# a-r-r-o-w/finetrainers

Measured on NVIDIA H100. Metric: latent_tokens_per_sec, higher is better.
Workload: dtype bf16

## Files before the change

finetrainers_b200/csrc/b2d_attn.cu:

```cuda
#include <stdlib.h>
#include <type_traits>
#include "b2d_internal.h"
#include "b2d_ptx.cuh"

namespace b2d {

constexpr int ATT_THREADS = 384;
constexpr int TILE = 128;
constexpr int PANEL = 64;
constexpr int TILE_PANEL_BYTES = TILE * PANEL * 2;
constexpr int HALF_PANEL_BYTES = 64 * PANEL * 2;
constexpr int ATT_SMEM_LIMIT = 227 * 1024;
constexpr float LOG2E = 1.4426950408889634f;
constexpr float LN2 = 0.6931471805599453f;

template <int HD>
struct AttnShape {
    static_assert(HD == 64 || HD == 128, "attention is built for head_dim 64 and 128");
    static constexpr int PANELS = HD / PANEL;
    static constexpr int TILE_BYTES = PANELS * TILE_PANEL_BYTES;
    static constexpr int HALF_BYTES = PANELS * HALF_PANEL_BYTES;
};

__device__ __forceinline__ float fast_exp2(float x) {
// ... 271 lines not shown
    const long long t = (long long)blockIdx.x * blockDim.x + threadIdx.x;
    const long long total = (long long)B * Sq * H * LANES;
    const bool ok = t < total;
    const long long e0 = (ok ? t : 0) * 8;
    uint4 a = *reinterpret_cast<const uint4*>(out + e0);
    uint4 d = *reinterpret_cast<const uint4*>(dout + e0);
    float acc = bf16_lo(a.x) * bf16_lo(d.x) + bf16_hi(a.x) * bf16_hi(d.x) + bf16_lo(a.y) * bf16_lo(d.y) +
                bf16_hi(a.y) * bf16_hi(d.y) + bf16_lo(a.z) * bf16_lo(d.z) + bf16_hi(a.z) * bf16_hi(d.z) +
                bf16_lo(a.w) * bf16_lo(d.w) + bf16_hi(a.w) * bf16_hi(d.w);
#pragma unroll
    for (int o = 1; o < LANES; o <<= 1) acc += __shfl_xor_sync(0xffffffffu, acc, o);
    if (ok && (t & (LANES - 1)) == 0) {
        const long long hr = t >> LOG2_LANES;
        const int h = (int)(hr % H);
        const long long bq = hr / H;
        const int q = (int)(bq % Sq);
        const int b = (int)(bq / Sq);
        const long long o = ((long long)b * H + h) * Sq + q;
        delta[o] = acc;
        nlse2[o] = -lse[o] * LOG2E;
    }
}

struct AttnBwdParams {
    CUtensorMap tmX1, tmX2, tmY1, tmY2;
    const float* key_bias;
    const float* delta;
    const float* nlse2;
    __nv_bfloat16* out1;
    __nv_bfloat16* out2;
    float* acc1;
    float* acc2;
    long long part_stride;
    int y_per_split;
    int B, H, Sq, Sk;
    float scale, scale_log2;
};

constexpr int BWD_STAGES = 4;
constexpr int ATT_MAX_SPLITS = 8;
template <int HD>
constexpr int BWD_SMEM = 2 * AttnShape<HD>::TILE_BYTES + BWD_STAGES * 2 * AttnShape<HD>::HALF_BYTES + 1024 + 256;
static_assert(BWD_SMEM<64> <= ATT_SMEM_LIMIT && BWD_SMEM<128> <= ATT_SMEM_LIMIT, "attn_bwd shared memory");
template <int HD>
constexpr int BWD_REGS_PRODUCER = HD == 64 ? 40 : 24;
template <int HD>
constexpr int BWD_REGS_MATH = HD == 64 ? 232 : 240;
static_assert(BWD_REGS_PRODUCER<64> * 128 + BWD_REGS_MATH<64> * 256 == 168 * ATT_THREADS &&
                  BWD_REGS_PRODUCER<128> * 128 + BWD_REGS_MATH<128> * 256 == 168 * ATT_THREADS,
              "setmaxnreg split");

template <bool DKV, int HD>
__global__ void __launch_bounds__(ATT_THREADS, 1) attn_bwd_kernel(const __grid_constant__ AttnBwdParams p) {
    constexpr int TILE_BYTES = AttnShape<HD>::TILE_BYTES, HALF_BYTES = AttnShape<HD>::HALF_BYTES;
    griddep_launch_dependents();
    extern __shared__ uint8_t smem_raw[];
    uint8_t* smem = reinterpret_cast<uint8_t*>((reinterpret_cast<uintptr_t>(smem_raw) + 1023) & ~uintptr_t(1023));
    uint8_t* sX = smem;
    uint8_t* sY = smem + 2 * TILE_BYTES;
    uint64_t* x_bar = reinterpret_cast<uint64_t*>(sY + BWD_STAGES * 2 * HALF_BYTES);
    uint64_t* full_bar = x_bar + 1;
    uint64_t* empty_bar = full_bar + BWD_STAGES;

    const int warp = threadIdx.x >> 5, lane = threadIdx.x & 31;
    const int xt = blockIdx.x, bh = blockIdx.y;
    const int b = bh / p.H, h = bh % p.H;
    const int S_x = DKV ? p.Sk : p.Sq, S_y = DKV ? p.Sq : p.Sk;
    const int n_y = (S_y + 63) / 64;
    const int y_begin = blockIdx.z * p.y_per_split;
    const int y_end = min(n_y, y_begin + p.y_per_split);

    if (threadIdx.x == 0) {
        tma_prefetch_desc(&p.tmX1);
        tma_prefetch_desc(&p.tmX2);
        tma_prefetch_desc(&p.tmY1);
        tma_prefetch_desc(&p.tmY2);
        mbar_init(x_bar, 1);
        for (int i = 0; i < BWD_STAGES; ++i) {
            mbar_init(&full_bar[i], 1);
            mbar_init(&empty_bar[i], 256);
        }
        fence_mbar_init();
    }
    __syncthreads();
    griddep_wait();

    if (warp < 4) {
        setmaxnreg_dec<BWD_REGS_PRODUCER<HD>>();
        if (warp == 0 && elect_one()) {
            mbar_expect_tx(x_bar, 2 * TILE_BYTES);
            tma_load_tile<HD, TILE_PANEL_BYTES>(sX, &p.tmX1, x_bar, h, xt * TILE, b);
            tma_load_tile<HD, TILE_PANEL_BYTES>(sX + TILE_BYTES, &p.tmX2, x_bar, h, xt * TILE, b);
            int stage = 0;
            uint32_t phase = 0;
            for (int y = y_begin; y < y_end; ++y) {
                mbar_wait(&empty_bar[stage], phase ^ 1);
                uint8_t* s1 = sY + stage * 2 * HALF_BYTES;
                mbar_expect_tx(&full_bar[stage], 2 * HALF_BYTES);
                tma_load_tile<HD, HALF_PANEL_BYTES>(s1, &p.tmY1, &full_bar[stage], h, y * 64, b);
                tma_load_tile<HD, HALF_PANEL_BYTES>(s1 + HALF_BYTES, &p.tmY2, &full_bar[stage], h, y * 64, b);
                if (++stage == BWD_STAGES) {
                    stage = 0;
                    phase ^= 1;
                }
            }
        }
        return;
    }
    setmaxnreg_inc<BWD_REGS_MATH<HD>>();
    const int cw = (warp >> 2) - 1, wq = warp & 3;
    const int qd = lane & 3;
    const uint32_t x1 = smem_u32(sX) + cw * HALF_PANEL_BYTES, x2 = x1 + TILE_BYTES;
    const float* kb = p.key_bias ? p.key_bias + (long long)b * p.Sk : nullptr;
    const float* nlse2 = p.nlse2 + (long long)bh * p.Sq;
    const float* delta = p.delta + (long long)bh * p.Sq;
    const int nq = p.B * p.H * p.Sq;
    auto neg_lse2 = [&](int q) { return HD == 64 ? nlse2[q] : delta[q + nq]; };
    const float sl2 = p.scale_log2;
    const int r0 = xt * TILE + cw * 64 + wq * 16 + (lane >> 2);

    float row_off[2], row_delta[2];
#pragma unroll
    for (int hh = 0; hh < 2; ++hh) {
        const int r = r0 + 8 * hh;
        if (DKV) {
            row_off[hh] = (kb != nullptr && r < p.Sk) ? kb[r] * LOG2E : 0.f;
            row_delta[hh] = 0.f;
        } else {
            row_off[hh] = r < p.Sq ? neg_lse2(r) : 0.f;
            row_delta[hh] = r < p.Sq ? delta[r] : 0.f;
        }
    }
    float acc1[HD / 2], acc2[HD / 2];
#pragma unroll
    for (int i = 0; i < HD / 2; ++i) acc1[i] = acc2[i] = 0.f;
    float c_off[16], c_delta[16];
    auto load_cols = [&](int y) {
#pragma unroll
        for (int k = 0; k < 16; ++k) {
            const int c = y * 64 + 8 * (k >> 1) + 2 * qd + (k & 1);
            const bool ok = c < S_y;
            if (DKV) {
                c_off[k] = ok ? neg_lse2(c) : 0.f;
                c_delta[k] = ok ? delta[c] : 0.f;
            } else {
                c_off[k] = (ok && kb != nullptr) ? kb[c] * LOG2E : 0.f;
            }
        }
    };
    float s[32], dp[32];
    auto elementwise = [&](int y, auto ragged) {
#pragma unroll
        for (int k = 0; k < 16; ++k) {
            const int jj = k >> 1, e = k & 1;
            const bool ok = !decltype(ragged)::value || y * 64 + 8 * jj + 2 * qd + e < S_y;
#pragma unroll
            for (int hh = 0; hh < 2; ++hh) {
                const int i = 4 * jj + 2 * hh + e;
                const float pr = ok ? fast_exp2(fmaf(s[i], sl2, row_off[hh] + c_off[k])) : 0.f;
                const float dl = DKV ? c_delta[k] : row_delta[hh];
                s[i] = pr;
                dp[i] = pr * (dp[i] - dl);
            }
        }
    };
    auto turn_begin = [&] { named_bar_sync(1 + cw, 256); };
    auto turn_end = [&](bool last) {
        if (cw == 0 || !last) named_bar_arrive(2 - cw, 256);
    };
    mbar_wait(x_bar, 0);
    if (cw == 1) named_bar_arrive(1, 256);
    int stage = 0;
    uint32_t phase = 0;
    for (int y = y_begin; y < y_end; ++y) {
        mbar_wait(&full_bar[stage], phase);
        const uint32_t y1 = smem_u32(sY + stage * 2 * HALF_BYTES), y2 = y1 + HALF_BYTES;
        turn_begin();
        wgmma_fence();
        mma_xyt<64, HD, TILE_PANEL_BYTES, HALF_PANEL_BYTES>(s, x1, y1);
        mma_xyt<64, HD, TILE_PANEL_BYTES, HALF_PANEL_BYTES>(dp, x2, y2);
        wgmma_commit();
        turn_end(false);
        if (HD == 64) load_cols(y);
        wgmma_wait<0>();
        wgmma_fence_regs(s);
        wgmma_fence_regs(dp);
        if (HD != 64) load_cols(y);
        if ((y + 1) * 64 > S_y)
            elementwise(y, std::true_type{});
        else
            elementwise(y, std::false_type{});
        uint32_t pa[4][4], da[4][4];
        acc_to_a<4>(dp, da);
        turn_begin();
        wgmma_fence();
        if (DKV) {
            acc_to_a<4>(s, pa);
            mma_az<4, HD, HALF_PANEL_BYTES>(acc1, pa, y2);
            mma_az<4, HD, HALF_PANEL_BYTES>(acc2, da, y1);
        } else {
            mma_az<4, HD, HALF_PANEL_BYTES>(acc2, da, y1);
        }
        wgmma_commit();
        turn_end(y + 1 == y_end);
        wgmma_wait<0>();
        wgmma_fence_regs(acc1);
        wgmma_fence_regs(acc2);
        mbar_arrive(&empty_bar[stage]);
        if (++stage == BWD_STAGES) {
            stage = 0;
            phase ^= 1;
        }
    }
#pragma unroll
    for (int hh = 0; hh < 2; ++hh) {
        const int r = r0 + 8 * hh;
        if (r >= S_x) continue;
        const long long base = ((long long)bh * S_x + r) * HD;
#pragma unroll
        for (int jj = 0; jj < HD / 8; ++jj) {
            const int c = 8 * jj + 2 * qd, i = 4 * jj + 2 * hh;
            const float g0 = acc2[i] * p.scale, g1 = acc2[i + 1] * p.scale;
            if (p.acc2 != nullptr) {
                const long long zoff = (long long)blockIdx.z * p.part_stride;
                *reinterpret_cast<float2*>(p.acc2 + zoff + base + c) = make_float2(g0, g1);
                if (DKV) *reinterpret_cast<float2*>(p.acc1 + zoff + base + c) = make_float2(acc1[i], acc1[i + 1]);
            } else {
                *reinterpret_cast<uint32_t*>(p.out2 + base + c) = pack_bf16x2(g0, g1);
                if (DKV) *reinterpret_cast<uint32_t*>(p.out1 + base + c) = pack_bf16x2(acc1[i], acc1[i + 1]);
            }
        }
    }
}

__global__ void attn_dkv_reduce_kernel(const float* __restrict__ part, int splits, long long stride, long long n,
                                       __nv_bfloat16* __restrict__ dv, __nv_bfloat16* __restrict__ dk) {
    griddep_launch_dependents();
    griddep_wait();
    const long long i = ((long long)blockIdx.x * blockDim.x + threadIdx.x) * 4;
    if (i + 3 >= 2 * n) return;
    float4 a = *reinterpret_cast<const float4*>(part + i);
    for (int z = 1; z < splits; ++z) {
        const float4 v = *reinterpret_cast<const float4*>(part + z * stride + i);
        a.x += v.x;
        a.y += v.y;
        a.z += v.z;
        a.w += v.w;
    }
    __nv_bfloat16* dst = i < n ? dv + i : dk + (i - n);
    *reinterpret_cast<uint2*>(dst) = make_uint2(pack_bf16x2(a.x, a.y), pack_bf16x2(a.z, a.w));
}

static int make_head_map(CUtensorMap* m, const void* base, int hd, int B, int H, int S, long long stride_h,
                         long long stride_s, long long stride_b, int box_rows = 128) {
// ... 21 lines not shown
    return 0;
}

template <int HD>
static int attn_fwd(const void* q, const void* k, const void* v, const float* key_bias, void* out, float* lse, int B,
                    int H, int Sq, int Sk, float scale, cudaStream_t st) {
    AttnFwdParams p;
    memset(&p, 0, sizeof(p));
    int rc;
    if ((rc = make_head_map(&p.tmQ, q, HD, B, H, Sq, (long long)Sq * HD, HD, (long long)H * Sq * HD))) return rc;
    if ((rc = make_head_map(&p.tmK, k, HD, B, H, Sk, (long long)Sk * HD, HD, (long long)H * Sk * HD))) return rc;
    if ((rc = make_head_map(&p.tmV, v, HD, B, H, Sk, (long long)Sk * HD, HD, (long long)H * Sk * HD))) return rc;
    p.key_bias = key_bias;
    p.out = (__nv_bfloat16*)out;
    p.lse = lse;
    p.B = B; p.H = H; p.Sq = Sq; p.Sk = Sk;
    p.scale_log2 = scale * LOG2E;
    if ((rc = set_smem((const void*)attn_fwd_kernel<HD>, FWD_SMEM<HD>, "attn_fwd"))) return rc;
    launch_k(attn_fwd_kernel<HD>, dim3((Sq + TILE - 1) / TILE, B * H), dim3(ATT_THREADS), FWD_SMEM<HD>, st, p);
    B2D_CHECK_LAUNCH("attn_fwd");
    return 0;
}

template <int HD>
static int attn_bwd(const void* q, const void* k, const void* v, const float* key_bias, const void* out,
                    const void* dout, const float* lse, float* delta_ws, void* dq, void* dk, void* dv, int B, int H,
                    int Sq, int Sk, float scale, cudaStream_t st) {
    {
        long long total = (long long)B * Sq * H * (HD / 8);
        launch_k(attn_delta_kernel<HD>, dim3((unsigned)((total + 255) / 256)), dim3(256), 0, st,
                 (const __nv_bfloat16*)out, (const __nv_bfloat16*)dout, lse, delta_ws, delta_ws + (long long)B * H * Sq,
                 B, H, Sq);
        B2D_CHECK_LAUNCH("attn_delta");
    }
    CUtensorMap mQ, mK, mV, mdO, mQy, mKy, mVy, mdOy;
    int rc;
    const long long hs_q = (long long)Sq * HD, hs_k = (long long)Sk * HD, tok = (long long)H * HD;
    if ((rc = make_head_map(&mQ, q, HD, B, H, Sq, hs_q, HD, H * hs_q))) return rc;
    if ((rc = make_head_map(&mK, k, HD, B, H, Sk, hs_k, HD, H * hs_k))) return rc;
    if ((rc = make_head_map(&mV, v, HD, B, H, Sk, hs_k, HD, H * hs_k))) return rc;
    if ((rc = make_head_map(&mdO, dout, HD, B, H, Sq, HD, tok, Sq * tok))) return rc;
    if ((rc = make_head_map(&mQy, q, HD, B, H, Sq, hs_q, HD, H * hs_q, 64))) return rc;
    if ((rc = make_head_map(&mKy, k, HD, B, H, Sk, hs_k, HD, H * hs_k, 64))) return rc;
    if ((rc = make_head_map(&mVy, v, HD, B, H, Sk, hs_k, HD, H * hs_k, 64))) return rc;
    if ((rc = make_head_map(&mdOy, dout, HD, B, H, Sq, HD, tok, Sq * tok, 64))) return rc;
    if ((rc = set_smem((const void*)attn_bwd_kernel<true, HD>, BWD_SMEM<HD>, "attn_bwd_dkv"))) return rc;
    if ((rc = set_smem((const void*)attn_bwd_kernel<false, HD>, BWD_SMEM<HD>, "attn_bwd_dq"))) return rc;
    AttnBwdParams p;
    memset(&p, 0, sizeof(p));
    p.key_bias = key_bias; p.delta = delta_ws; p.nlse2 = delta_ws + (long long)B * H * Sq;
    p.B = B; p.H = H; p.Sq = Sq; p.Sk = Sk;
    p.scale = scale; p.scale_log2 = scale * LOG2E;
    p.tmX1 = mK; p.tmX2 = mV; p.tmY1 = mQy; p.tmY2 = mdOy;
    p.out1 = (__nv_bfloat16*)dv; p.out2 = (__nv_bfloat16*)dk;
    const int n_yq = (Sq + 63) / 64;
    const int kv_ctas = ((Sk + TILE - 1) / TILE) * B * H;
    const int nsm = device_sm_count();
    if (nsm <= 0) return B2D_ERR_CUDA;
    int splits = 1;
    if (Sk <= 512 && kv_ctas < nsm && n_yq >= 8) splits = min(ATT_MAX_SPLITS, min(n_yq / 4, (nsm + kv_ctas - 1) / kv_ctas));
    p.y_per_split = (n_yq + splits - 1) / splits;
    splits = (n_yq + p.y_per_split - 1) / p.y_per_split;
    if (splits > 1) {
        const long long n_kv = (long long)B * H * Sk * HD;
        p.acc1 = delta_ws + 2LL * B * H * Sq;
        p.acc2 = p.acc1 + n_kv;
        p.part_stride = 2 * n_kv;
        launch_k(attn_bwd_kernel<true, HD>, dim3((Sk + TILE - 1) / TILE, B * H, splits), dim3(ATT_THREADS), BWD_SMEM<HD>,
                 st, p);
        B2D_CHECK_LAUNCH("attn_bwd_dkv(split)");
        launch_k(attn_dkv_reduce_kernel, dim3((unsigned)((2 * n_kv / 4 + 255) / 256)), dim3(256), 0, st, (const float*)p.acc1,
                 splits, 2 * n_kv, n_kv, (__nv_bfloat16*)dv, (__nv_bfloat16*)dk);
        B2D_CHECK_LAUNCH("attn_bwd_dkv(reduce)");
    } else {
        launch_k(attn_bwd_kernel<true, HD>, dim3((Sk + TILE - 1) / TILE, B * H), dim3(ATT_THREADS), BWD_SMEM<HD>, st, p);
        B2D_CHECK_LAUNCH("attn_bwd_dkv");
    }
    p.acc1 = p.acc2 = nullptr;
    p.tmX1 = mQ; p.tmX2 = mdO; p.tmY1 = mKy; p.tmY2 = mVy;
    p.out1 = nullptr; p.out2 = (__nv_bfloat16*)dq;
    p.y_per_split = (Sk + 63) / 64;
    launch_k(attn_bwd_kernel<false, HD>, dim3((Sq + TILE - 1) / TILE, B * H), dim3(ATT_THREADS), BWD_SMEM<HD>, st, p);
    B2D_CHECK_LAUNCH("attn_bwd_dq");
    return 0;
}

}

using namespace b2d;

extern "C" int b2d_attn_fwd_hd(const void* q, const void* k, const void* v, const float* key_bias, void* out, float* lse,
                               int32_t B, int32_t H, int32_t Sq, int32_t Sk, int32_t head_dim, float scale,
                               void* stream) {
    B2D_BIND(q);
    if (B <= 0 || H <= 0 || Sq <= 0 || Sk <= 0) return set_error(B2D_ERR_SHAPE, "attn_fwd: bad dims");
    if (head_dim != 64 && head_dim != 128)
        return set_error(B2D_ERR_SHAPE, "attn_fwd: head_dim %d is not supported (64 or 128)", (int)head_dim);
    if (reinterpret_cast<uintptr_t>(out) & 31) return set_error(B2D_ERR_ALIGN, "attn_fwd: out must be 32-byte aligned");
    cudaStream_t st = reinterpret_cast<cudaStream_t>(stream);
    return head_dim == 64 ? b2d::attn_fwd<64>(q, k, v, key_bias, out, lse, B, H, Sq, Sk, scale, st)
                          : b2d::attn_fwd<128>(q, k, v, key_bias, out, lse, B, H, Sq, Sk, scale, st);
}

extern "C" int b2d_attn_bwd_hd(const void* q, const void* k, const void* v, const float* key_bias, const void* out,
                               const void* dout, const float* lse, float* delta_ws, void* dq, void* dk, void* dv,
                               int32_t B, int32_t H, int32_t Sq, int32_t Sk, int32_t head_dim, float scale,
                               void* stream) {
    B2D_BIND(q);
    if (B <= 0 || H <= 0 || Sq <= 0 || Sk <= 0) return set_error(B2D_ERR_SHAPE, "attn_bwd: bad dims");
    if (head_dim != 64 && head_dim != 128)
        return set_error(B2D_ERR_SHAPE, "attn_bwd: head_dim %d is not supported (64 or 128)", (int)head_dim);
    cudaStream_t st = reinterpret_cast<cudaStream_t>(stream);
    return head_dim == 64
               ? b2d::attn_bwd<64>(q, k, v, key_bias, out, dout, lse, delta_ws, dq, dk, dv, B, H, Sq, Sk, scale, st)
               : b2d::attn_bwd<128>(q, k, v, key_bias, out, dout, lse, delta_ws, dq, dk, dv, B, H, Sq, Sk, scale, st);
}

extern "C" int b2d_attn_fwd(const void* q, const void* k, const void* v, const float* key_bias, void* out, float* lse,
                            int32_t B, int32_t H, int32_t Sq, int32_t Sk, float scale, void* stream) {
    return b2d_attn_fwd_hd(q, k, v, key_bias, out, lse, B, H, Sq, Sk, 64, scale, stream);
}

extern "C" int b2d_attn_bwd(const void* q, const void* k, const void* v, const float* key_bias, const void* out,
                            const void* dout, const float* lse, float* delta_ws, void* dq, void* dk, void* dv,
                            int32_t B, int32_t H, int32_t Sq, int32_t Sk, float scale, void* stream) {
    return b2d_attn_bwd_hd(q, k, v, key_bias, out, dout, lse, delta_ws, dq, dk, dv, B, H, Sq, Sk, 64, scale, stream);
}
```

finetrainers_b200/lib.py:

```python
from __future__ import annotations

import ctypes as C
import os
import subprocess
import threading

_HERE = os.path.dirname(os.path.abspath(__file__))
LIB_PATH = os.path.join(_HERE, "libb2d.so")
_lib = None
_lock = threading.Lock()


class B2DError(RuntimeError):
    pass


class GemmDesc(C.Structure):
    _fields_ = [
        ("A", C.c_void_p), ("lda", C.c_int64),
        ("B", C.c_void_p), ("ldb", C.c_int64),
        ("A2", C.c_void_p), ("lda2", C.c_int64),
        ("B2", C.c_void_p), ("ldb2", C.c_int64),
        ("M", C.c_int32), ("N", C.c_int32), ("K", C.c_int32), ("K2", C.c_int32),
        ("a_mn_major", C.c_int32), ("b_mn_major", C.c_int32),
# ... 45 lines not shown
        if not os.path.exists(LIB_PATH):
            try:
                build()
            except Exception as e:
                raise B2DError(f"{LIB_PATH} not found and building it failed ({e}); there is no CPU or PyTorch "
                               "fallback for the b200 hot path") from e
        lib = C.CDLL(LIB_PATH)
        lib.b2d_last_error.restype = C.c_char_p
        lib.b2d_version.restype = C.c_int
        _lib = lib
    return _lib


def check(rc: int, what: str = ""):
    if rc != 0:
        msg = load().b2d_last_error().decode()
        raise B2DError(f"libb2d {what} failed (code {rc}): {msg}")


EXPORTS = [
    "b2d_version", "b2d_last_error", "b2d_device_check", "b2d_gemm",
    "b2d_norm_modulate_fwd", "b2d_norm_modulate_bwd", "b2d_colscale",
    "b2d_qknorm_rope_fwd", "b2d_qknorm_rope_bwd", "b2d_qkv_norm_rope_fwd", "b2d_qkv_norm_rope_bwd", "b2d_rope_table",
    "b2d_attn_fwd", "b2d_attn_bwd", "b2d_attn_fwd_hd", "b2d_attn_bwd_hd",
    "b2d_prep_noise_pack", "b2d_loss_mse", "b2d_timestep_sinusoid", "b2d_cast_f32_bf16",
    "b2d_sumsq", "b2d_adamw_clip", "b2d_upcast_fp8_bf16",
]
```

finetrainers_b200/ops.py:

```python
from __future__ import annotations

import ctypes as C
from typing import Optional

import torch

from . import lib as _l
from .lib import GemmDesc, check

EPI_STORE, EPI_GELU, EPI_SILU, EPI_GATE_RES, EPI_MUL_DGELU, EPI_F32_ATOMIC, EPI_F32_ATOMIC_T, EPI_F32_STORE = range(8)

LAUNCH_COUNT = 0
TIMING = False
KERNEL_TIMES = {}
CONTEXT = ""


class _Timed:
    __slots__ = ("tag", "e0")

    def __init__(self, tag):
        self.tag = tag

    def __enter__(self):
# ... 147 lines not shown
              "qkv_norm_rope_bwd")
    _count()
    return dx


def rope_table(cos, sin, F, H, W, D, sf, sh, sw):
    check(_l.load().b2d_rope_table(_ptr(cos), _ptr(sin), F, H, W, D, C.c_float(sf), C.c_float(sh), C.c_float(sw),
                                   _stream()), "rope_table")
    _count()


def attn_fwd(q, k, v, key_bias, out, lse, B, H, Sq, Sk, scale, *, head_dim=64):
    with _Timed("attn_fwd"):
        check(_l.load().b2d_attn_fwd_hd(_ptr(q), _ptr(k), _ptr(v), _ptr(key_bias), _ptr(out), _ptr(lse), B, H, Sq, Sk,
                                        head_dim, C.c_float(scale), _stream()), "attn_fwd")
    _count()
    return out


def attn_bwd_ws_floats(B, H, Sq, Sk, *, head_dim=64):
    return 2 * B * H * Sq + (8 * 2 * B * H * Sk * head_dim if Sk <= 512 else 0)


def attn_bwd(q, k, v, key_bias, out, dout, lse, delta_ws, dq, dk, dv, B, H, Sq, Sk, scale, *, head_dim=64):
    need = attn_bwd_ws_floats(B, H, Sq, Sk, head_dim=head_dim)
    if delta_ws.numel() < need:
        raise _l.B2DError(f"attn_bwd workspace too small: {delta_ws.numel()} < {need} floats")
    with _Timed("attn_bwd"):
        check(_l.load().b2d_attn_bwd_hd(_ptr(q), _ptr(k), _ptr(v), _ptr(key_bias), _ptr(out), _ptr(dout), _ptr(lse),
                                        _ptr(delta_ws), _ptr(dq), _ptr(dk), _ptr(dv), B, H, Sq, Sk, head_dim,
                                        C.c_float(scale), _stream()), "attn_bwd")
    if Sk <= 128:
        _count(1)
    else:
        split = (B * H * ((Sk + 127) // 128) < 96) and Sk <= 512 and ((Sq + 63) // 64) >= 8
        _count(5 if split else 3)


def prep_noise_pack(latents, noise, mean, std, sigma, sigma_ff, x_t, target, B, Cc, F, HW):
    check(_l.load().b2d_prep_noise_pack(_ptr(latents), _ptr(noise), _ptr(mean), _ptr(std), _ptr(sigma),
                                        _ptr(sigma_ff), _ptr(x_t), _ptr(target), B, Cc, F, HW, _stream()), "prep")
    _count()


def loss_mse(pred, target, weight, loss_scale, loss_out, dpred, partial_ws, B, per_sample):
    with _Timed("loss"):
        check(_l.load().b2d_loss_mse(_ptr(pred), _ptr(target), _ptr(weight), C.c_float(loss_scale), _ptr(loss_out),
                                     _ptr(dpred), _ptr(partial_ws), B, C.c_int64(per_sample), _stream()), "loss_mse")
    _count(2)


def timestep_sinusoid(t, out, n):
    check(_l.load().b2d_timestep_sinusoid(_ptr(t), _ptr(out), n, _stream()), "timestep_sinusoid")
    _count()


def cast_f32_bf16(src, dst, n, scale=1.0):
    with _Timed("cast"):
        check(_l.load().b2d_cast_f32_bf16(_ptr(src), _ptr(dst), C.c_int64(n), C.c_float(scale), _stream()), "cast")
# ... 28 lines not shown
```

include/b2d.h:

```cpp
#ifndef B2D_H
#define B2D_H
#include <stddef.h>
#include <stdint.h>
#ifdef __cplusplus
extern "C" {
#endif

typedef enum {
  B2D_OK = 0,
  B2D_ERR_SHAPE = -1,
  B2D_ERR_ALIGN = -2,
  B2D_ERR_ARCH = -3,
  B2D_ERR_CUDA = -4,
  B2D_ERR_ARG = -5
} b2d_status;

int b2d_version(void);
const char* b2d_last_error(void);
int b2d_device_check(void);

typedef enum {
  B2D_EPI_STORE = 0,
  B2D_EPI_GELU = 1,
  B2D_EPI_SILU = 2,
// ... 49 lines not shown
int b2d_qknorm_rope_fwd(const void* src, int64_t ld, int64_t col_off, const void* weight, const void* cos,
                        const void* sin, void* dst, int32_t B, int32_t S, int32_t H, int32_t norm, float eps,
                        void* stream);
int b2d_qknorm_rope_bwd(const void* dsrc_heads, const void* x, int64_t ld, int64_t col_off, const void* weight,
                        const void* cos, const void* sin, void* dx, int64_t ld_dx, int64_t dx_col_off, int32_t B,
                        int32_t S, int32_t H, int32_t norm, float eps, void* stream);
int b2d_qkv_norm_rope_fwd(const void* src, int64_t ld, int64_t col_off, int32_t nseg, const void* w0, const void* w1,
                          const void* w2, int32_t rope_mask, const void* cos, const void* sin, void* dst0, void* dst1,
                          void* dst2, int32_t B, int32_t S, int32_t H, float eps, int32_t rows_per_w, int64_t w_stride,
                          void* stream);
int b2d_qkv_norm_rope_bwd(const void* dy0, const void* dy1, const void* dy2, const void* x, int64_t ld, int64_t col_off,
                          int32_t nseg, const void* w0, const void* w1, const void* w2, int32_t rope_mask, const void* cos,
                          const void* sin, void* dx, int64_t ld_dx, int64_t dx_col_off, int32_t B, int32_t S, int32_t H,
                          float eps, int32_t rows_per_w, int64_t w_stride, void* stream);

int b2d_rope_table(float* cos, float* sin, int32_t F, int32_t H, int32_t W, int32_t D, float sf, float sh, float sw,
                   void* stream);

int b2d_attn_fwd_hd(const void* q, const void* k, const void* v, const float* key_bias, void* out, float* lse,
                    int32_t B, int32_t H, int32_t Sq, int32_t Sk, int32_t head_dim, float scale, void* stream);
int b2d_attn_bwd_hd(const void* q, const void* k, const void* v, const float* key_bias, const void* out,
                    const void* dout, const float* lse, float* delta_ws, void* dq, void* dk, void* dv, int32_t B,
                    int32_t H, int32_t Sq, int32_t Sk, int32_t head_dim, float scale, void* stream);
int b2d_attn_fwd(const void* q, const void* k, const void* v, const float* key_bias, void* out, float* lse, int32_t B,
                 int32_t H, int32_t Sq, int32_t Sk, float scale, void* stream);
int b2d_attn_bwd(const void* q, const void* k, const void* v, const float* key_bias, const void* out, const void* dout,
                 const float* lse, float* delta_ws, void* dq, void* dk, void* dv, int32_t B, int32_t H, int32_t Sq,
                 int32_t Sk, float scale, void* stream);

#define B2D_REDUCE_PARTIALS 296
int b2d_prep_noise_pack(const void* latents, const void* noise, const float* mean, const float* std,
                        const float* sigma, const float* sigma_ff, void* x_t, void* target, int32_t B, int32_t C,
                        int32_t F, int32_t HW, void* stream);
int b2d_loss_mse(const void* pred, const void* target, const float* weight, float loss_scale, float* loss_out,
                 void* dpred, float* partial_ws, int32_t B, int64_t per_sample, void* stream);

int b2d_timestep_sinusoid(const float* t, void* out, int32_t n, void* stream);

int b2d_cast_f32_bf16(const float* src, void* dst, int64_t n, float scale, void* stream);

int b2d_upcast_fp8_bf16(const void* src, void* dst, int64_t n, int32_t fmt, void* stream);

int b2d_sumsq(const float* x, int64_t n, float* out_sumsq , float* partial_ws, void* stream);
int b2d_adamw_clip(float* p, float* g, float* m, float* v, int64_t n, const float* sumsq, float max_norm, float lr,
                   float beta1, float beta2, float eps, float wd, int32_t step, float grad_div, void* stream);

// ... 5 lines not shown
```

Baseline: 36270.

## Merge attention backward dKV and dQ passes into one persistent scheduled kernel

Replaces the separate dK/dV and dQ backward launches with a single persistent kernel that walks a static per-CTA schedule of dKV and dQ work items. The host picks a skip parameter by a makespan cost model so the tail is balanced. For head_dim 64 the X tile is double-buffered so the next item's load overlaps the current one. The goal is fewer launches and better SM load balance, at the cost of more complex barrier phase tracking and extra shared memory.

New measurement: 37340, median of 6. +3.0%, better.

```diff
diff --git a/finetrainers_b200/csrc/b2d_attn.cu b/finetrainers_b200/csrc/b2d_attn.cu
--- a/finetrainers_b200/csrc/b2d_attn.cu
+++ b/finetrainers_b200/csrc/b2d_attn.cu
@@ -1,4 +1,5 @@
 #include <stdlib.h>
+#include <algorithm>
 #include <type_traits>
 #include "b2d_internal.h"
 #include "b2d_ptx.cuh"
@@ -317,17 +318,31 @@
     }
 }
 
+__host__ __device__ __forceinline__ int bwd_sched_item(int G, int n_kv, int n_dq, int skip, int cta, int t) {
+    const int r = n_kv % G;
+    const int a = cta < n_kv ? (n_kv - 1 - cta) / G + 1 : 0;
+    if (t < a) return cta + t * G;
+    const int k = t - a + (cta < r ? skip : 0);
+    const int m = k < skip ? k * (G - r) + cta - r : skip * (G - r) + (k - skip) * G + cta;
+    return m < n_dq ? n_kv + m : -1;
+}
+
 struct AttnBwdParams {
-    CUtensorMap tmX1, tmX2, tmY1, tmY2;
+    CUtensorMap tmK, tmV, tmQy, tmdOy;
+    CUtensorMap tmQ, tmdO, tmKy, tmVy;
     const float* key_bias;
     const float* delta;
     const float* nlse2;
-    __nv_bfloat16* out1;
-    __nv_bfloat16* out2;
-    float* acc1;
-    float* acc2;
+    __nv_bfloat16* dq;
+    __nv_bfloat16* dk;
+    __nv_bfloat16* dv;
+    float* acc_dv;
+    float* acc_dk;
     long long part_stride;
     int y_per_split;
+    int kv_tiles, q_tiles;
+    int n_kv, n_dq;
+    int skip;
     int B, H, Sq, Sk;
     float scale, scale_log2;
 };
@@ -335,7 +350,10 @@
 constexpr int BWD_STAGES = 4;
 constexpr int ATT_MAX_SPLITS = 8;
 template <int HD>
-constexpr int BWD_SMEM = 2 * AttnShape<HD>::TILE_BYTES + BWD_STAGES * 2 * AttnShape<HD>::HALF_BYTES + 1024 + 256;
+constexpr int BWD_XBUFS = HD == 64 ? 2 : 1;
+template <int HD>
+constexpr int BWD_SMEM =
+    BWD_XBUFS<HD> * 2 * AttnShape<HD>::TILE_BYTES + BWD_STAGES * 2 * AttnShape<HD>::HALF_BYTES + 1024 + 256;
 static_assert(BWD_SMEM<64> <= ATT_SMEM_LIMIT && BWD_SMEM<128> <= ATT_SMEM_LIMIT, "attn_bwd shared memory");
 template <int HD>
 constexpr int BWD_REGS_PRODUCER = HD == 64 ? 40 : 24;
@@ -345,32 +363,62 @@
                   BWD_REGS_PRODUCER<128> * 128 + BWD_REGS_MATH<128> * 256 == 168 * ATT_THREADS,
               "setmaxnreg split");
 
-template <bool DKV, int HD>
+struct BwdItem {
+    bool dkv;
+    int xt, bh, z, y_begin, y_end;
+};
+__device__ __forceinline__ BwdItem bwd_decode(const AttnBwdParams& p, int it) {
+    BwdItem w;
+    w.dkv = it < p.n_kv;
+    if (w.dkv) {
+        w.xt = it % p.kv_tiles;
+        const int rest = it / p.kv_tiles, bhs = p.B * p.H;
+        w.bh = rest % bhs;
+        w.z = rest / bhs;
+        w.y_begin = w.z * p.y_per_split;
+        w.y_end = min((p.Sq + 63) / 64, w.y_begin + p.y_per_split);
+    } else {
+        const int m = it - p.n_kv;
+        w.xt = m % p.q_tiles;
+        w.bh = m / p.q_tiles;
+        w.z = 0;
+        w.y_begin = 0;
+        w.y_end = (p.Sk + 63) / 64;
+    }
+    return w;
+}
+
+template <bool SPLIT, int HD>
 __global__ void __launch_bounds__(ATT_THREADS, 1) attn_bwd_kernel(const __grid_constant__ AttnBwdParams p) {
     constexpr int TILE_BYTES = AttnShape<HD>::TILE_BYTES, HALF_BYTES = AttnShape<HD>::HALF_BYTES;
+    constexpr int XBUFS = BWD_XBUFS<HD>;
     griddep_launch_dependents();
     extern __shared__ uint8_t smem_raw[];
     uint8_t* smem = reinterpret_cast<uint8_t*>((reinterpret_cast<uintptr_t>(smem_raw) + 1023) & ~uintptr_t(1023));
     uint8_t* sX = smem;
-    uint8_t* sY = smem + 2 * TILE_BYTES;
-    uint64_t* x_bar = reinterpret_cast<uint64_t*>(sY + BWD_STAGES * 2 * HALF_BYTES);
-    uint64_t* full_bar = x_bar + 1;
+    uint8_t* sY = smem + XBUFS * 2 * TILE_BYTES;
+    uint64_t* xfull_bar = reinterpret_cast<uint64_t*>(sY + BWD_STAGES * 2 * HALF_BYTES);
+    uint64_t* xempty_bar = xfull_bar + XBUFS;
+    uint64_t* full_bar = xempty_bar + XBUFS;
     uint64_t* empty_bar = full_bar + BWD_STAGES;
 
     const int warp = threadIdx.x >> 5, lane = threadIdx.x & 31;
-    const int xt = blockIdx.x, bh = blockIdx.y;
-    const int b = bh / p.H, h = bh % p.H;
-    const int S_x = DKV ? p.Sk : p.Sq, S_y = DKV ? p.Sq : p.Sk;
-    const int n_y = (S_y + 63) / 64;
-    const int y_begin = blockIdx.z * p.y_per_split;
-    const int y_end = min(n_y, y_begin + p.y_per_split);
+    const int G = gridDim.x, cta = blockIdx.x;
+    auto item_of = [&](int t) { return bwd_sched_item(G, p.n_kv, p.n_dq, p.skip, cta, t); };
 
     if (threadIdx.x == 0) {
-        tma_prefetch_desc(&p.tmX1);
-        tma_prefetch_desc(&p.tmX2);
-        tma_prefetch_desc(&p.tmY1);
-        tma_prefetch_desc(&p.tmY2);
-        mbar_init(x_bar, 1);
+        tma_prefetch_desc(&p.tmK);
+        tma_prefetch_desc(&p.tmV);
+        tma_prefetch_desc(&p.tmQy);
+        tma_prefetch_desc(&p.tmdOy);
+        tma_prefetch_desc(&p.tmQ);
+        tma_prefetch_desc(&p.tmdO);
+        tma_prefetch_desc(&p.tmKy);
+        tma_prefetch_desc(&p.tmVy);
+        for (int i = 0; i < XBUFS; ++i) {
+            mbar_init(&xfull_bar[i], 1);
+            mbar_init(&xempty_bar[i], 256);
+        }
         for (int i = 0; i < BWD_STAGES; ++i) {
             mbar_init(&full_bar[i], 1);
             mbar_init(&empty_bar[i], 256);
@@ -383,20 +431,32 @@
     if (warp < 4) {
         setmaxnreg_dec<BWD_REGS_PRODUCER<HD>>();
         if (warp == 0 && elect_one()) {
-            mbar_expect_tx(x_bar, 2 * TILE_BYTES);
-            tma_load_tile<HD, TILE_PANEL_BYTES>(sX, &p.tmX1, x_bar, h, xt * TILE, b);
-            tma_load_tile<HD, TILE_PANEL_BYTES>(sX + TILE_BYTES, &p.tmX2, x_bar, h, xt * TILE, b);
             int stage = 0;
             uint32_t phase = 0;
-            for (int y = y_begin; y < y_end; ++y) {
-                mbar_wait(&empty_bar[stage], phase ^ 1);
-                uint8_t* s1 = sY + stage * 2 * HALF_BYTES;
-                mbar_expect_tx(&full_bar[stage], 2 * HALF_BYTES);
-                tma_load_tile<HD, HALF_PANEL_BYTES>(s1, &p.tmY1, &full_bar[stage], h, y * 64, b);
-                tma_load_tile<HD, HALF_PANEL_BYTES>(s1 + HALF_BYTES, &p.tmY2, &full_bar[stage], h, y * 64, b);
-                if (++stage == BWD_STAGES) {
-                    stage = 0;
-                    phase ^= 1;
+            for (int t = 0;; ++t) {
+                const int it = item_of(t);
+                if (it < 0) break;
+                const BwdItem w = bwd_decode(p, it);
+                const int b = w.bh / p.H, h = w.bh % p.H;
+                const int xb = t % XBUFS;
+                uint8_t* x = sX + xb * 2 * TILE_BYTES;
+                mbar_wait(&xempty_bar[xb], ((t / XBUFS) & 1) ^ 1);
+                mbar_expect_tx(&xfull_bar[xb], 2 * TILE_BYTES);
+                tma_load_tile<HD, TILE_PANEL_BYTES>(x, w.dkv ? &p.tmK : &p.tmQ, &xfull_bar[xb], h, w.xt * TILE, b);
+                tma_load_tile<HD, TILE_PANEL_BYTES>(x + TILE_BYTES, w.dkv ? &p.tmV : &p.tmdO, &xfull_bar[xb], h,
+                                                    w.xt * TILE, b);
+                const CUtensorMap* my1 = w.dkv ? &p.tmQy : &p.tmKy;
+                const CUtensorMap* my2 = w.dkv ? &p.tmdOy : &p.tmVy;
+                for (int y = w.y_begin; y < w.y_end; ++y) {
+                    mbar_wait(&empty_bar[stage], phase ^ 1);
+                    uint8_t* s1 = sY + stage * 2 * HALF_BYTES;
+                    mbar_expect_tx(&full_bar[stage], 2 * HALF_BYTES);
+                    tma_load_tile<HD, HALF_PANEL_BYTES>(s1, my1, &full_bar[stage], h, y * 64, b);
+                    tma_load_tile<HD, HALF_PANEL_BYTES>(s1 + HALF_BYTES, my2, &full_bar[stage], h, y * 64, b);
+                    if (++stage == BWD_STAGES) {
+                        stage = 0;
+                        phase ^= 1;
+                    }
                 }
             }
         }
@@ -405,126 +465,148 @@
     setmaxnreg_inc<BWD_REGS_MATH<HD>>();
     const int cw = (warp >> 2) - 1, wq = warp & 3;
     const int qd = lane & 3;
-    const uint32_t x1 = smem_u32(sX) + cw * HALF_PANEL_BYTES, x2 = x1 + TILE_BYTES;
-    const float* kb = p.key_bias ? p.key_bias + (long long)b * p.Sk : nullptr;
-    const float* nlse2 = p.nlse2 + (long long)bh * p.Sq;
-    const float* delta = p.delta + (long long)bh * p.Sq;
-    const int nq = p.B * p.H * p.Sq;
-    auto neg_lse2 = [&](int q) { return HD == 64 ? nlse2[q] : delta[q + nq]; };
     const float sl2 = p.scale_log2;
-    const int r0 = xt * TILE + cw * 64 + wq * 16 + (lane >> 2);
-
-    float row_off[2], row_delta[2];
-#pragma unroll
-    for (int hh = 0; hh < 2; ++hh) {
-        const int r = r0 + 8 * hh;
-        if (DKV) {
-            row_off[hh] = (kb != nullptr && r < p.Sk) ? kb[r] * LOG2E : 0.f;
-            row_delta[hh] = 0.f;
-        } else {
-            row_off[hh] = r < p.Sq ? neg_lse2(r) : 0.f;
-            row_delta[hh] = r < p.Sq ? delta[r] : 0.f;
-        }
-    }
-    float acc1[HD / 2], acc2[HD / 2];
-#pragma unroll
-    for (int i = 0; i < HD / 2; ++i) acc1[i] = acc2[i] = 0.f;
-    float c_off[16], c_delta[16];
-    auto load_cols = [&](int y) {
-#pragma unroll
-        for (int k = 0; k < 16; ++k) {
-            const int c = y * 64 + 8 * (k >> 1) + 2 * qd + (k & 1);
-            const bool ok = c < S_y;
-            if (DKV) {
-                c_off[k] = ok ? neg_lse2(c) : 0.f;
-                c_delta[k] = ok ? delta[c] : 0.f;
-            } else {
-                c_off[k] = (ok && kb != nullptr) ? kb[c] * LOG2E : 0.f;
-            }
-        }
-    };
-    float s[32], dp[32];
-    auto elementwise = [&](int y, auto ragged) {
-#pragma unroll
-        for (int k = 0; k < 16; ++k) {
-            const int jj = k >> 1, e = k & 1;
-            const bool ok = !decltype(ragged)::value || y * 64 + 8 * jj + 2 * qd + e < S_y;
-#pragma unroll
-            for (int hh = 0; hh < 2; ++hh) {
-                const int i = 4 * jj + 2 * hh + e;
-                const float pr = ok ? fast_exp2(fmaf(s[i], sl2, row_off[hh] + c_off[k])) : 0.f;
-                const float dl = DKV ? c_delta[k] : row_delta[hh];
-                s[i] = pr;
-                dp[i] = pr * (dp[i] - dl);
-            }
-        }
-    };
     auto turn_begin = [&] { named_bar_sync(1 + cw, 256); };
     auto turn_end = [&](bool last) {
         if (cw == 0 || !last) named_bar_arrive(2 - cw, 256);
     };
-    mbar_wait(x_bar, 0);
-    if (cw == 1) named_bar_arrive(1, 256);
     int stage = 0;
     uint32_t phase = 0;
-    for (int y = y_begin; y < y_end; ++y) {
-        mbar_wait(&full_bar[stage], phase);
-        const uint32_t y1 = smem_u32(sY + stage * 2 * HALF_BYTES), y2 = y1 + HALF_BYTES;
-        turn_begin();
-        wgmma_fence();
-        mma_xyt<64, HD, TILE_PANEL_BYTES, HALF_PANEL_BYTES>(s, x1, y1);
-        mma_xyt<64, HD, TILE_PANEL_BYTES, HALF_PANEL_BYTES>(dp, x2, y2);
-        wgmma_commit();
-        turn_end(false);
-        if (HD == 64) load_cols(y);
-        wgmma_wait<0>();
-        wgmma_fence_regs(s);
-        wgmma_fence_regs(dp);
-        if (HD != 64) load_cols(y);
-        if ((y + 1) * 64 > S_y)
-            elementwise(y, std::true_type{});
+
+    auto run_item = [&](auto dkv_tag, const BwdItem& w, int xb, uint32_t xphase, bool last_item) {
+        constexpr bool DKV = decltype(dkv_tag)::value;
+        const int bh = w.bh, b = bh / p.H;
+        const int S_x = DKV ? p.Sk : p.Sq, S_y = DKV ? p.Sq : p.Sk;
+        const int y_begin = w.y_begin, y_end = w.y_end;
+        const uint32_t x1 = smem_u32(sX + xb * 2 * TILE_BYTES) + cw * HALF_PANEL_BYTES, x2 = x1 + TILE_BYTES;
+        const float* kb = p.key_bias ? p.key_bias + (long long)b * p.Sk : nullptr;
+        const float* nlse2 = p.nlse2 + (long long)bh * p.Sq;
+        const float* delta = p.delta + (long long)bh * p.Sq;
+        const int nq = p.B * p.H * p.Sq;
+        auto neg_lse2 = [&](int q) { return HD == 64 ? nlse2[q] : delta[q + nq]; };
+        const int r0 = w.xt * TILE + cw * 64 + wq * 16 + (lane >> 2);
+
+        float row_off[2], row_delta[2];
+#pragma unroll
+        for (int hh = 0; hh < 2; ++hh) {
+            const int r = r0 + 8 * hh;
+            if (DKV) {
+                row_off[hh] = (kb != nullptr && r < p.Sk) ? kb[r] * LOG2E : 0.f;
+                row_delta[hh] = 0.f;
+            } else {
+                row_off[hh] = r < p.Sq ? neg_lse2(r) : 0.f;
+                row_delta[hh] = r < p.Sq ? delta[r] : 0.f;
+            }
+        }
+        float acc1[HD / 2], acc2[HD / 2];
+#pragma unroll
+        for (int i = 0; i < HD / 2; ++i) acc1[i] = acc2[i] = 0.f;
+        float c_off[16], c_delta[16];
+        auto load_cols = [&](int y) {
+#pragma unroll
+            for (int k = 0; k < 16; ++k) {
+                const int c = y * 64 + 8 * (k >> 1) + 2 * qd + (k & 1);
+                const bool ok = c < S_y;
+                if (DKV) {
+                    c_off[k] = ok ? neg_lse2(c) : 0.f;
+                    c_delta[k] = ok ? delta[c] : 0.f;
+                } else {
+                    c_off[k] = (ok && kb != nullptr) ? kb[c] * LOG2E : 0.f;
+                }
+            }
+        };
+        float s[32], dp[32];
+        auto elementwise = [&](int y, auto ragged) {
+#pragma unroll
+            for (int k = 0; k < 16; ++k) {
+                const int jj = k >> 1, e = k & 1;
+                const bool ok = !decltype(ragged)::value || y * 64 + 8 * jj + 2 * qd + e < S_y;
+#pragma unroll
+                for (int hh = 0; hh < 2; ++hh) {
+                    const int i = 4 * jj + 2 * hh + e;
+                    const float pr = ok ? fast_exp2(fmaf(s[i], sl2, row_off[hh] + c_off[k])) : 0.f;
+                    const float dl = DKV ? c_delta[k] : row_delta[hh];
+                    s[i] = pr;
+                    dp[i] = pr * (dp[i] - dl);
+                }
+            }
+        };
+        mbar_wait(&xfull_bar[xb], xphase);
+        for (int y = y_begin; y < y_end; ++y) {
+            mbar_wait(&full_bar[stage], phase);
+            const uint32_t y1 = smem_u32(sY + stage * 2 * HALF_BYTES), y2 = y1 + HALF_BYTES;
+            turn_begin();
+            wgmma_fence();
+            mma_xyt<64, HD, TILE_PANEL_BYTES, HALF_PANEL_BYTES>(s, x1, y1);
+            mma_xyt<64, HD, TILE_PANEL_BYTES, HALF_PANEL_BYTES>(dp, x2, y2);
+            wgmma_commit();
+            turn_end(false);
+            if (HD == 64) load_cols(y);
+            wgmma_wait<0>();
+            wgmma_fence_regs(s);
+            wgmma_fence_regs(dp);
+            if (y + 1 == y_end) mbar_arrive(&xempty_bar[xb]);
+            if (HD != 64) load_cols(y);
+            if ((y + 1) * 64 > S_y)
+                elementwise(y, std::true_type{});
+            else
+                elementwise(y, std::false_type{});
+            uint32_t pa[4][4], da[4][4];
+            acc_to_a<4>(dp, da);
+            turn_begin();
+            wgmma_fence();
+            if (DKV) {
+                acc_to_a<4>(s, pa);
+                mma_az<4, HD, HALF_PANEL_BYTES>(acc1, pa, y2);
+                mma_az<4, HD, HALF_PANEL_BYTES>(acc2, da, y1);
+            } else {
+                mma_az<4, HD, HALF_PANEL_BYTES>(acc2, da, y1);
+            }
+            wgmma_commit();
+            turn_end(last_item && y + 1 == y_end);
+            wgmma_wait<0>();
+            wgmma_fence_regs(acc1);
+            wgmma_fence_regs(acc2);
+            mbar_arrive(&empty_bar[stage]);
+            if (++stage == BWD_STAGES) {
+                stage = 0;
+                phase ^= 1;
+            }
+        }
+        __nv_bfloat16* out1 = p.dv;
+        __nv_bfloat16* out2 = DKV ? p.dk : p.dq;
+#pragma unroll
+        for (int hh = 0; hh < 2; ++hh) {
+            const int r = r0 + 8 * hh;
+            if (r >= S_x) continue;
+            const long long base = ((long long)bh * S_x + r) * HD;
+#pragma unroll
+            for (int jj = 0; jj < HD / 8; ++jj) {
+                const int c = 8 * jj + 2 * qd, i = 4 * jj + 2 * hh;
+                const float g0 = acc2[i] * p.scale, g1 = acc2[i + 1] * p.scale;
+                if (DKV && SPLIT) {
+                    const long long zoff = (long long)w.z * p.part_stride;
+                    *reinterpret_cast<float2*>(p.acc_dk + zoff + base + c) = make_float2(g0, g1);
+                    *reinterpret_cast<float2*>(p.acc_dv + zoff + base + c) = make_float2(acc1[i], acc1[i + 1]);
+                } else {
+                    *reinterpret_cast<uint32_t*>(out2 + base + c) = pack_bf16x2(g0, g1);
+                    if (DKV) *reinterpret_cast<uint32_t*>(out1 + base + c) = pack_bf16x2(acc1[i], acc1[i + 1]);
+                }
+            }
+        }
+    };
+
+    int it = item_of(0);
+    if (cw == 1 && it >= 0) named_bar_arrive(1, 256);
+    for (int t = 0; it >= 0; ++t) {
+        const int next = item_of(t + 1);
+        const BwdItem w = bwd_decode(p, it);
+        const uint32_t xphase = (t / XBUFS) & 1;
+        if (w.dkv)
+            run_item(std::true_type{}, w, t % XBUFS, xphase, next < 0);
         else
-            elementwise(y, std::false_type{});
-        uint32_t pa[4][4], da[4][4];
-        acc_to_a<4>(dp, da);
-        turn_begin();
-        wgmma_fence();
-        if (DKV) {
-            acc_to_a<4>(s, pa);
-            mma_az<4, HD, HALF_PANEL_BYTES>(acc1, pa, y2);
-            mma_az<4, HD, HALF_PANEL_BYTES>(acc2, da, y1);
-        } else {
-            mma_az<4, HD, HALF_PANEL_BYTES>(acc2, da, y1);
-        }
-        wgmma_commit();
-        turn_end(y + 1 == y_end);
-        wgmma_wait<0>();
-        wgmma_fence_regs(acc1);
-        wgmma_fence_regs(acc2);
-        mbar_arrive(&empty_bar[stage]);
-        if (++stage == BWD_STAGES) {
-            stage = 0;
-            phase ^= 1;
-        }
-    }
-#pragma unroll
-    for (int hh = 0; hh < 2; ++hh) {
-        const int r = r0 + 8 * hh;
-        if (r >= S_x) continue;
-        const long long base = ((long long)bh * S_x + r) * HD;
-#pragma unroll
-        for (int jj = 0; jj < HD / 8; ++jj) {
-            const int c = 8 * jj + 2 * qd, i = 4 * jj + 2 * hh;
-            const float g0 = acc2[i] * p.scale, g1 = acc2[i + 1] * p.scale;
-            if (p.acc2 != nullptr) {
-                const long long zoff = (long long)blockIdx.z * p.part_stride;
-                *reinterpret_cast<float2*>(p.acc2 + zoff + base + c) = make_float2(g0, g1);
-                if (DKV) *reinterpret_cast<float2*>(p.acc1 + zoff + base + c) = make_float2(acc1[i], acc1[i + 1]);
-            } else {
-                *reinterpret_cast<uint32_t*>(p.out2 + base + c) = pack_bf16x2(g0, g1);
-                if (DKV) *reinterpret_cast<uint32_t*>(p.out1 + base + c) = pack_bf16x2(acc1[i], acc1[i + 1]);
-            }
-        }
+            run_item(std::false_type{}, w, t % XBUFS, xphase, next < 0);
+        it = next;
     }
 }
 
@@ -592,10 +674,26 @@
     return 0;
 }
 
+static long long bwd_item_cost(bool dkv, int y_tiles) { return (dkv ? 4LL : 3LL) * y_tiles + 2; }
+
+static long long bwd_sched_makespan(int G, int n_kv, int n_dq, int skip, long long c_kv, long long c_dq) {
+    const int r = n_kv % G, lo = G - r;
+    long long worst = 0;
+    for (int cta = 0; cta < G; ++cta) {
+        const long long a = cta < n_kv ? (n_kv - 1 - cta) / G + 1 : 0;
+        long long m = 0;
+        if (cta >= r && skip > 0 && n_dq > cta - r) m += min(skip, (n_dq - (cta - r) + lo - 1) / lo);
+        const long long first = (long long)skip * lo + cta;
+        if (n_dq > first) m += (n_dq - first - 1) / G + 1;
+        worst = std::max(worst, a * c_kv + m * c_dq);
+    }
+    return worst;
+}
+
 template <int HD>
 static int attn_bwd(const void* q, const void* k, const void* v, const float* key_bias, const void* out,
                     const void* dout, const float* lse, float* delta_ws, void* dq, void* dk, void* dv, int B, int H,
-                    int Sq, int Sk, float scale, cudaStream_t st) {
+                    int Sq, int Sk, float scale, int max_ctas, cudaStream_t st) {
     {
         long long total = (long long)B * Sq * H * (HD / 8);
         launch_k(attn_delta_kernel<HD>, dim3((unsigned)((total + 255) / 256)), dim3(256), 0, st,
@@ -603,55 +701,62 @@
                  B, H, Sq);
         B2D_CHECK_LAUNCH("attn_delta");
     }
-    CUtensorMap mQ, mK, mV, mdO, mQy, mKy, mVy, mdOy;
+    AttnBwdParams p;
+    memset(&p, 0, sizeof(p));
     int rc;
     const long long hs_q = (long long)Sq * HD, hs_k = (long long)Sk * HD, tok = (long long)H * HD;
-    if ((rc = make_head_map(&mQ, q, HD, B, H, Sq, hs_q, HD, H * hs_q))) return rc;
-    if ((rc = make_head_map(&mK, k, HD, B, H, Sk, hs_k, HD, H * hs_k))) return rc;
-    if ((rc = make_head_map(&mV, v, HD, B, H, Sk, hs_k, HD, H * hs_k))) return rc;
-    if ((rc = make_head_map(&mdO, dout, HD, B, H, Sq, HD, tok, Sq * tok))) return rc;
-    if ((rc = make_head_map(&mQy, q, HD, B, H, Sq, hs_q, HD, H * hs_q, 64))) return rc;
-    if ((rc = make_head_map(&mKy, k, HD, B, H, Sk, hs_k, HD, H * hs_k, 64))) return rc;
-    if ((rc = make_head_map(&mVy, v, HD, B, H, Sk, hs_k, HD, H * hs_k, 64))) return rc;
-    if ((rc = make_head_map(&mdOy, dout, HD, B, H, Sq, HD, tok, Sq * tok, 64))) return rc;
-    if ((rc = set_smem((const void*)attn_bwd_kernel<true, HD>, BWD_SMEM<HD>, "attn_bwd_dkv"))) return rc;
-    if ((rc = set_smem((const void*)attn_bwd_kernel<false, HD>, BWD_SMEM<HD>, "attn_bwd_dq"))) return rc;
-    AttnBwdParams p;
-    memset(&p, 0, sizeof(p));
+    if ((rc = make_head_map(&p.tmQ, q, HD, B, H, Sq, hs_q, HD, H * hs_q))) return rc;
+    if ((rc = make_head_map(&p.tmK, k, HD, B, H, Sk, hs_k, HD, H * hs_k))) return rc;
+    if ((rc = make_head_map(&p.tmV, v, HD, B, H, Sk, hs_k, HD, H * hs_k))) return rc;
+    if ((rc = make_head_map(&p.tmdO, dout, HD, B, H, Sq, HD, tok, Sq * tok))) return rc;
+    if ((rc = make_head_map(&p.tmQy, q, HD, B, H, Sq, hs_q, HD, H * hs_q, 64))) return rc;
+    if ((rc = make_head_map(&p.tmKy, k, HD, B, H, Sk, hs_k, HD, H * hs_k, 64))) return rc;
+    if ((rc = make_head_map(&p.tmVy, v, HD, B, H, Sk, hs_k, HD, H * hs_k, 64))) return rc;
+    if ((rc = make_head_map(&p.tmdOy, dout, HD, B, H, Sq, HD, tok, Sq * tok, 64))) return rc;
     p.key_bias = key_bias; p.delta = delta_ws; p.nlse2 = delta_ws + (long long)B * H * Sq;
+    p.dq = (__nv_bfloat16*)dq; p.dk = (__nv_bfloat16*)dk; p.dv = (__nv_bfloat16*)dv;
     p.B = B; p.H = H; p.Sq = Sq; p.Sk = Sk;
     p.scale = scale; p.scale_log2 = scale * LOG2E;
-    p.tmX1 = mK; p.tmX2 = mV; p.tmY1 = mQy; p.tmY2 = mdOy;
-    p.out1 = (__nv_bfloat16*)dv; p.out2 = (__nv_bfloat16*)dk;
-    const int n_yq = (Sq + 63) / 64;
-    const int kv_ctas = ((Sk + TILE - 1) / TILE) * B * H;
+    const int n_yq = (Sq + 63) / 64, n_yk = (Sk + 63) / 64;
+    p.kv_tiles = (Sk + TILE - 1) / TILE;
+    p.q_tiles = (Sq + TILE - 1) / TILE;
+    const int kv_ctas = p.kv_tiles * B * H;
     const int nsm = device_sm_count();
     if (nsm <= 0) return B2D_ERR_CUDA;
     int splits = 1;
     if (Sk <= 512 && kv_ctas < nsm && n_yq >= 8) splits = min(ATT_MAX_SPLITS, min(n_yq / 4, (nsm + kv_ctas - 1) / kv_ctas));
     p.y_per_split = (n_yq + splits - 1) / splits;
     splits = (n_yq + p.y_per_split - 1) / p.y_per_split;
+    const long long n_kvel = (long long)B * H * Sk * HD;
     if (splits > 1) {
-        const long long n_kv = (long long)B * H * Sk * HD;
-        p.acc1 = delta_ws + 2LL * B * H * Sq;
-        p.acc2 = p.acc1 + n_kv;
-        p.part_stride = 2 * n_kv;
-        launch_k(attn_bwd_kernel<true, HD>, dim3((Sk + TILE - 1) / TILE, B * H, splits), dim3(ATT_THREADS), BWD_SMEM<HD>,
-                 st, p);
-        B2D_CHECK_LAUNCH("attn_bwd_dkv(split)");
-        launch_k(attn_dkv_reduce_kernel, dim3((unsigned)((2 * n_kv / 4 + 255) / 256)), dim3(256), 0, st, (const float*)p.acc1,
-                 splits, 2 * n_kv, n_kv, (__nv_bfloat16*)dv, (__nv_bfloat16*)dk);
-        B2D_CHECK_LAUNCH("attn_bwd_dkv(reduce)");
+        p.acc_dv = delta_ws + 2LL * B * H * Sq;
+        p.acc_dk = p.acc_dv + n_kvel;
+        p.part_stride = 2 * n_kvel;
+    }
+    p.n_kv = kv_ctas * splits;
+    p.n_dq = p.q_tiles * B * H;
+    const int G = min(max_ctas > 0 ? max_ctas : nsm, p.n_kv + p.n_dq);
+    const long long c_kv = bwd_item_cost(true, p.y_per_split), c_dq = bwd_item_cost(false, n_yk);
+    long long best = -1;
+    for (int skip = 0; skip <= c_kv / c_dq + 1; ++skip) {
+        const long long t = bwd_sched_makespan(G, p.n_kv, p.n_dq, skip, c_kv, c_dq);
+        if (best < 0 || t < best) {
+            best = t;
+            p.skip = skip;
+        }
+    }
+    if (splits > 1) {
+        if ((rc = set_smem((const void*)attn_bwd_kernel<true, HD>, BWD_SMEM<HD>, "attn_bwd(split)"))) return rc;
+        launch_k(attn_bwd_kernel<true, HD>, dim3(G), dim3(ATT_THREADS), BWD_SMEM<HD>, st, p);
+        B2D_CHECK_LAUNCH("attn_bwd(split)");
+        launch_k(attn_dkv_reduce_kernel, dim3((unsigned)((2 * n_kvel / 4 + 255) / 256)), dim3(256), 0, st,
+                 (const float*)p.acc_dv, splits, 2 * n_kvel, n_kvel, (__nv_bfloat16*)dv, (__nv_bfloat16*)dk);
+        B2D_CHECK_LAUNCH("attn_bwd(reduce)");
     } else {
-        launch_k(attn_bwd_kernel<true, HD>, dim3((Sk + TILE - 1) / TILE, B * H), dim3(ATT_THREADS), BWD_SMEM<HD>, st, p);
-        B2D_CHECK_LAUNCH("attn_bwd_dkv");
-    }
-    p.acc1 = p.acc2 = nullptr;
-    p.tmX1 = mQ; p.tmX2 = mdO; p.tmY1 = mKy; p.tmY2 = mVy;
-    p.out1 = nullptr; p.out2 = (__nv_bfloat16*)dq;
-    p.y_per_split = (Sk + 63) / 64;
-    launch_k(attn_bwd_kernel<false, HD>, dim3((Sq + TILE - 1) / TILE, B * H), dim3(ATT_THREADS), BWD_SMEM<HD>, st, p);
-    B2D_CHECK_LAUNCH("attn_bwd_dq");
+        if ((rc = set_smem((const void*)attn_bwd_kernel<false, HD>, BWD_SMEM<HD>, "attn_bwd"))) return rc;
+        launch_k(attn_bwd_kernel<false, HD>, dim3(G), dim3(ATT_THREADS), BWD_SMEM<HD>, st, p);
+        B2D_CHECK_LAUNCH("attn_bwd");
+    }
     return 0;
 }
 
@@ -672,18 +777,27 @@
                           : b2d::attn_fwd<128>(q, k, v, key_bias, out, lse, B, H, Sq, Sk, scale, st);
 }
 
-extern "C" int b2d_attn_bwd_hd(const void* q, const void* k, const void* v, const float* key_bias, const void* out,
-                               const void* dout, const float* lse, float* delta_ws, void* dq, void* dk, void* dv,
-                               int32_t B, int32_t H, int32_t Sq, int32_t Sk, int32_t head_dim, float scale,
-                               void* stream) {
+extern "C" int b2d_attn_bwd_grid(const void* q, const void* k, const void* v, const float* key_bias, const void* out,
+                                 const void* dout, const float* lse, float* delta_ws, void* dq, void* dk, void* dv,
+                                 int32_t B, int32_t H, int32_t Sq, int32_t Sk, int32_t head_dim, float scale,
+                                 int32_t max_ctas, void* stream) {
     B2D_BIND(q);
     if (B <= 0 || H <= 0 || Sq <= 0 || Sk <= 0) return set_error(B2D_ERR_SHAPE, "attn_bwd: bad dims");
     if (head_dim != 64 && head_dim != 128)
         return set_error(B2D_ERR_SHAPE, "attn_bwd: head_dim %d is not supported (64 or 128)", (int)head_dim);
     cudaStream_t st = reinterpret_cast<cudaStream_t>(stream);
-    return head_dim == 64
-               ? b2d::attn_bwd<64>(q, k, v, key_bias, out, dout, lse, delta_ws, dq, dk, dv, B, H, Sq, Sk, scale, st)
-               : b2d::attn_bwd<128>(q, k, v, key_bias, out, dout, lse, delta_ws, dq, dk, dv, B, H, Sq, Sk, scale, st);
+    return head_dim == 64 ? b2d::attn_bwd<64>(q, k, v, key_bias, out, dout, lse, delta_ws, dq, dk, dv, B, H, Sq, Sk,
+                                              scale, max_ctas, st)
+                          : b2d::attn_bwd<128>(q, k, v, key_bias, out, dout, lse, delta_ws, dq, dk, dv, B, H, Sq, Sk,
+                                               scale, max_ctas, st);
+}
+
+extern "C" int b2d_attn_bwd_hd(const void* q, const void* k, const void* v, const float* key_bias, const void* out,
+                               const void* dout, const float* lse, float* delta_ws, void* dq, void* dk, void* dv,
+                               int32_t B, int32_t H, int32_t Sq, int32_t Sk, int32_t head_dim, float scale,
+                               void* stream) {
+    return b2d_attn_bwd_grid(q, k, v, key_bias, out, dout, lse, delta_ws, dq, dk, dv, B, H, Sq, Sk, head_dim, scale, 0,
+                             stream);
 }
 
 extern "C" int b2d_attn_fwd(const void* q, const void* k, const void* v, const float* key_bias, void* out, float* lse,
diff --git a/finetrainers_b200/lib.py b/finetrainers_b200/lib.py
--- a/finetrainers_b200/lib.py
+++ b/finetrainers_b200/lib.py
@@ -91,7 +91,7 @@
     "b2d_version", "b2d_last_error", "b2d_device_check", "b2d_gemm",
     "b2d_norm_modulate_fwd", "b2d_norm_modulate_bwd", "b2d_colscale",
     "b2d_qknorm_rope_fwd", "b2d_qknorm_rope_bwd", "b2d_qkv_norm_rope_fwd", "b2d_qkv_norm_rope_bwd", "b2d_rope_table",
-    "b2d_attn_fwd", "b2d_attn_bwd", "b2d_attn_fwd_hd", "b2d_attn_bwd_hd",
+    "b2d_attn_fwd", "b2d_attn_bwd", "b2d_attn_fwd_hd", "b2d_attn_bwd_hd", "b2d_attn_bwd_grid",
     "b2d_prep_noise_pack", "b2d_loss_mse", "b2d_timestep_sinusoid", "b2d_cast_f32_bf16",
     "b2d_sumsq", "b2d_adamw_clip", "b2d_upcast_fp8_bf16",
 ]
diff --git a/finetrainers_b200/ops.py b/finetrainers_b200/ops.py
--- a/finetrainers_b200/ops.py
+++ b/finetrainers_b200/ops.py
@@ -193,19 +193,25 @@
     return 2 * B * H * Sq + (8 * 2 * B * H * Sk * head_dim if Sk <= 512 else 0)
 
 
-def attn_bwd(q, k, v, key_bias, out, dout, lse, delta_ws, dq, dk, dv, B, H, Sq, Sk, scale, *, head_dim=64):
+def attn_bwd_splits(B, H, Sq, Sk, n_sm):
+    n_yq, kv_tiles = (Sq + 63) // 64, B * H * ((Sk + 127) // 128)
+    if Sk > 512 or kv_tiles >= n_sm or n_yq < 8:
+        return 1
+    s = min(8, n_yq // 4, -(-n_sm // kv_tiles))
+    per = -(-n_yq // s)
+    return -(-n_yq // per)
+
+
+def attn_bwd(q, k, v, key_bias, out, dout, lse, delta_ws, dq, dk, dv, B, H, Sq, Sk, scale, *, head_dim=64, max_ctas=0):
     need = attn_bwd_ws_floats(B, H, Sq, Sk, head_dim=head_dim)
     if delta_ws.numel() < need:
         raise _l.B2DError(f"attn_bwd workspace too small: {delta_ws.numel()} < {need} floats")
     with _Timed("attn_bwd"):
-        check(_l.load().b2d_attn_bwd_hd(_ptr(q), _ptr(k), _ptr(v), _ptr(key_bias), _ptr(out), _ptr(dout), _ptr(lse),
-                                        _ptr(delta_ws), _ptr(dq), _ptr(dk), _ptr(dv), B, H, Sq, Sk, head_dim,
-                                        C.c_float(scale), _stream()), "attn_bwd")
-    if Sk <= 128:
-        _count(1)
-    else:
-        split = (B * H * ((Sk + 127) // 128) < 96) and Sk <= 512 and ((Sq + 63) // 64) >= 8
-        _count(5 if split else 3)
+        check(_l.load().b2d_attn_bwd_grid(_ptr(q), _ptr(k), _ptr(v), _ptr(key_bias), _ptr(out), _ptr(dout), _ptr(lse),
+                                          _ptr(delta_ws), _ptr(dq), _ptr(dk), _ptr(dv), B, H, Sq, Sk, head_dim,
+                                          C.c_float(scale), int(max_ctas), _stream()), "attn_bwd")
+    n_sm = torch.cuda.get_device_properties(q.device).multi_processor_count
+    _count(3 if attn_bwd_splits(B, H, Sq, Sk, n_sm) > 1 else 2)
 
 
 def prep_noise_pack(latents, noise, mean, std, sigma, sigma_ff, x_t, target, B, Cc, F, HW):
diff --git a/include/b2d.h b/include/b2d.h
--- a/include/b2d.h
+++ b/include/b2d.h
@@ -95,6 +95,9 @@
 int b2d_attn_bwd_hd(const void* q, const void* k, const void* v, const float* key_bias, const void* out,
                     const void* dout, const float* lse, float* delta_ws, void* dq, void* dk, void* dv, int32_t B,
                     int32_t H, int32_t Sq, int32_t Sk, int32_t head_dim, float scale, void* stream);
+int b2d_attn_bwd_grid(const void* q, const void* k, const void* v, const float* key_bias, const void* out,
+                      const void* dout, const float* lse, float* delta_ws, void* dq, void* dk, void* dv, int32_t B,
+                      int32_t H, int32_t Sq, int32_t Sk, int32_t head_dim, float scale, int32_t max_ctas, void* stream);
 int b2d_attn_fwd(const void* q, const void* k, const void* v, const float* key_bias, void* out, float* lse, int32_t B,
                  int32_t H, int32_t Sq, int32_t Sk, float scale, void* stream);
 int b2d_attn_bwd(const void* q, const void* k, const void* v, const float* key_bias, const void* out, const void* dout,
```
